# ysig/diff-mining

Measured on AMD Instinct MI355X. Metric: typicality-scored images/sec/node (512px, 10 t×2 prompts), higher is better.
Workload: dtype f16

## Files before the change

diff-mining_amd/csrc/igemm_pers_tr.hip:

```cpp
#include "igemm_pers_tile.h"

namespace dm {

namespace {

typedef volatile __attribute__((address_space(3))) int* lds_word_t;

template <int EXTRA, int WIMG, bool UNROLL = false, bool UP = false>
__global__ __launch_bounds__(512, 2)
void igemm_pers_tr_kernel(IGemmParams p, int ntiles, int cset) {
    constexpr int WC = 2, CH = 2, NW = 8;
    constexpr int TP = PERS_TP, TC = PERS_TC;
    constexpr int WBYTES = TC * 128;
    constexpr int PITCH = WIMG + 2;
    constexpr int IROWS = TP / WIMG;
    constexpr int ROWS = IROWS * PITCH;
    constexpr int XP = (ROWS + 7) / 8;
    constexpr int XBYTES = XP * 1024;
    constexpr int XI = (XP + NW - 1) / NW;
    constexpr int WI = TC / 8 / NW;
    constexpr int AUX_BYTES = 2048;
    constexpr bool GNBK = (EXTRA == PX_TEMB) && WIMG == 64;
    constexpr int NSTORE = pers_nstore(EPI_PLAIN, GNBK);
    static_assert(XI == 5 && 2 * WBYTES + 2 * XBYTES + 2 * AUX_BYTES <= 160 * 1024, "LDS budget");
    extern __shared__ __attribute__((aligned(16))) char smem[];
    char* const xs0 = smem + 2 * WBYTES;
    char* const aux0 = xs0 + 2 * XBYTES;

    const int wid = __builtin_amdgcn_readfirstlane(threadIdx.x >> 6);
    const int wc = wid % WC;
    const int wp = wid / WC;

    const int tiles_c = p.Cout / TC;
    int tile, tend, tdyn;
    const int xcd = blockIdx.x & 7;
    {
        const int nblk = gridDim.x;
        const int loc = blockIdx.x >> 3;
        const int tstart = xcd_range_start(blockIdx.x, ntiles);
        tend = tstart + (ntiles >> 3) + (xcd < (ntiles & 7) ? 1 : 0);
        tdyn = tstart + ((nblk - xcd + 7) >> 3);
        tile = tstart + loc;
    }
    int* const ctr = p.tile_ctr ? p.tile_ctr : &g_tile_ctr[cset][0];
    if (tile >= tend) { tiles_finish(ctr); return; }

    const int C1 = p.C1;
    const int C2 = p.Cin - C1;
    const int cpt = p.Cin / BK;
    const int ntrip = 3 * cpt;
    const int Ktot = 9 * p.Cin;
    const int OHW = p.OH * p.OW;

    int lp0 = 0, lc0 = 0;
    unsigned woff = 0;
    const unsigned wstride = (unsigned)(NW * 8) * (unsigned)Ktot;
    const f16* xbase = p.X;
    int ld_dy = 0, ld_cc = 0;

    auto set_wtile = [&](int tl) __attribute__((always_inline)) {
        const int pt = tl / tiles_c;
        lc0 = (tl - pt * tiles_c) * TC;
        const int ln = hw_lane();
        const int lrow = ln >> 3, lchunk = ((ln & 7) ^ lrow) * 8;
        woff = (unsigned)((size_t)(lc0 + wid * 8 + lrow) * Ktot + lchunk);
    };
    auto set_xtile = [&](int tl) __attribute__((always_inline)) {
        lp0 = (tl / tiles_c) * TP;
        ld_dy = 0; ld_cc = 0;
    };
    int x_dy = 0, x_cs = 0, x_cho = 0;
    auto src_pixel = [&](int i, int lrow) __attribute__((always_inline)) -> int {
        const int n = lp0 / OHW;
        const int oh0 = (lp0 - n * OHW) / WIMG;
        const int r = (wid + i * NW) * 8 + lrow;
        const int ir = r / PITCH;
        const int iw = r - ir * PITCH - 1;
        const int ih = oh0 + ir + x_dy - 1;
        if constexpr (UP) {
            const bool oku = r < ROWS && iw >= 0 && iw < WIMG && ih >= 0 && ih < p.OH;
            return oku ? (n * p.H + (ih >> 1)) * p.W + (iw >> 1) : -1;
        }
        const bool ok = r < ROWS && iw >= 0 && iw < WIMG && ih >= 0 && ih < p.H;
        return ok ? (n * p.H + ih) * WIMG + iw : -1;
    };
    auto prepare_x = [&]() __attribute__((always_inline)) {
        x_dy = ld_dy;
        const int ch = ld_cc * BK;
        if (ch < C1) { xbase = p.X; x_cs = C1; x_cho = ch; } else { xbase = p.X2; x_cs = C2; x_cho = ch - C1; }
        if (++ld_cc == cpt) { ld_cc = 0; ++ld_dy; }
    };
    auto load_w = [&](int buf, int idx, int adv) __attribute__((always_inline)) {
        lptr_t dst = (lptr_t)(smem + buf * WBYTES + (wid + idx * NW) * 1024);
        __builtin_amdgcn_global_load_lds((gptr_t)(p.Wp + (size_t)(woff + (unsigned)idx * wstride)), dst, 16, 0, 0);
        if (idx == WI - 1) woff += (unsigned)adv;
    };
    auto x_offset = [&](int i, int ln) __attribute__((always_inline)) -> int {
        const int lrow = ln >> 3, lchunk = ((ln & 7) ^ lrow) * 8;
        const int pix = src_pixel(i, lrow);
        return pix >= 0 ? pix * x_cs + x_cho + lchunk : -1;
    };
    auto load_x = [&](int buf, int i, int off, int ln) __attribute__((always_inline)) {
        if (i == XI - 1 && wid >= XP - NW * (XI - 1)) return;
        lptr_t dst = (lptr_t)(xs0 + buf * XBYTES + (wid + i * NW) * 1024);
        const f16* a = (off >= 0) ? (xbase + (size_t)(unsigned)off)
                                  : reinterpret_cast<const f16*>(p.zero_page) + lds_chunk(ln);
        __builtin_amdgcn_global_load_lds((gptr_t)a, dst, 16, 0, 0);
    };
    auto load_aux = [&](int slot, int lc0, int lp0) __attribute__((always_inline)) {
        char* ax = aux0 + slot * AUX_BYTES;
        const int lane = hw_lane();
        const char* zp = reinterpret_cast<const char*>(p.zero_page) + lane * 16;
        (void)load_aux_bias_temb<EXTRA>(p, ax, wid, lane, zp, lc0, lp0, OHW);
    };

    floatx4 acc[CH][5][4];

    constexpr bool SNAKE = DM_MFMA_SNAKE && !(EXTRA == PX_TEMB && WIMG == 64 && UNROLL);
    auto step = [&](int wcur, int xcur, auto dxv, int adv) __attribute__((always_inline)) {
        const int dx = dxv;
        const char* wt = smem + wcur * WBYTES;
        const char* xt = xs0 + xcur * XBYTES;
        const int ln = hw_lane();
        const int l15 = ln & 15, lg = ln >> 4;
        const int a_row_off = (wc * 80 * CH + l15) * 128;
        const int koff0 = ((lg ^ (l15 & 7)) << 4), koff1 = (((4 + lg) ^ (l15 & 7)) << 4);
        const int rb = ((wp * 64) / WIMG) * PITCH + (wp * 64) % WIMG + dx + l15;
        int boff[4];
#pragma unroll
        for (int j = 0; j < 4; ++j) {
            const int cj = ((16 * j) / WIMG) * PITCH + (16 * j) % WIMG;
            if (j > 0 && (cj & 7) == 0) { boff[j] = boff[0] + cj * 128; continue; }
            const int row = rb + cj;
            boff[j] = row * 128 + ((lg ^ (row & 7)) << 4);
        }
        half8 b0[4], b1[4], a[5];
#pragma unroll
        for (int j = 0; j < 4; ++j) b0[j] = *reinterpret_cast<const half8*>(xt + boff[j]);
#pragma unroll
        for (int i = 0; i < 5; ++i) a[i] = *reinterpret_cast<const half8*>(wt + a_row_off + i * 2048 + koff0);
        int grp = 0;
#pragma unroll
        for (int q = 0; q < 2 * CH; ++q) {
            const int sidx = q / CH, h = q % CH;
            if (q == CH - 1) {
#pragma unroll
                for (int j = 0; j < 4; ++j) {
                    const int cj = ((16 * j) / WIMG) * PITCH + (16 * j) % WIMG;
                    const int o1 = (j > 0 && (cj & 7) == 0) ? (boff[0] ^ 64) + cj * 128 : (boff[j] ^ 64);
                    b1[j] = *reinterpret_cast<const half8*>(xt + o1);
                }
            }
#pragma unroll
            for (int i = 0; i < 5; ++i) {
#pragma unroll
                for (int jj = 0; jj < 4; ++jj) {
                    const int j = (SNAKE && !(i & 1)) ? 3 - jj : jj;
                    acc[h][i][j] = __builtin_amdgcn_mfma_f32_16x16x32_f16(a[i], sidx ? b1[j] : b0[j], acc[h][i][j], 0, 0, 0);
                }
                if (q + 1 < 2 * CH) {
                    const int nq = q + 1, ns = nq / CH, nh = nq % CH;
                    a[i] = *reinterpret_cast<const half8*>(wt + a_row_off + nh * (80 * 128) + i * 2048 + (ns ? koff1 : koff0));
                }
                if (grp == 0) { load_w(wcur ^ 1, 0, adv); load_w(wcur ^ 1, 1, adv); }
                if (grp == 1) { load_w(wcur ^ 1, 2, adv); load_w(wcur ^ 1, 3, adv); }
                if (grp == 2) { load_w(wcur ^ 1, 4, adv); load_x(xcur ^ 1, 2 * dx, x_offset(2 * dx, ln), ln); }
                if (grp == 3) { if (dx < 2) load_x(xcur ^ 1, 2 * dx + 1, x_offset(2 * dx + 1, ln), ln); }
                ++grp;
                __builtin_amdgcn_sched_barrier(0);
            }
        }
    };

    set_wtile(tile);
    set_xtile(tile);
    load_aux(0, lc0, lp0);
    prepare_x();
    {
        const int ln = hw_lane();
#pragma unroll
        for (int i = 0; i < WI; ++i) load_w(0, i, p.Cin);
#pragma unroll
        for (int i = 0; i < XI; ++i) load_x(0, i, x_offset(i, ln), ln);
    }
    prepare_x();

    int g = 0;
    int tg = 0;
    int slot = 0;
    bool first = true;
    while (true) {
        const int pt = tile / tiles_c;
        const int p0 = pt * TP, c0out = (tile - pt * tiles_c) * TC;
#pragma unroll
        for (int h = 0; h < CH; ++h)
#pragma unroll
            for (int i = 0; i < 5; ++i)
#pragma unroll
                for (int j = 0; j < 4; ++j) acc[h][i][j] = floatx4{0.f, 0.f, 0.f, 0.f};

        if (first) wait_vmcnt_barrier<0>();
        else wait_vmcnt_barrier<NSTORE>();
        first = false;
        int ticket = 0;
        auto thread0 = [&]() __attribute__((always_inline)) -> bool {
            if constexpr (GNBK) return wid == 0 && hw_lane() == 0;
            else return threadIdx.x == 0;
        };
        if (thread0()) ticket = atomicAdd(&ctr[xcd * 32], 1);
        int next = 0;
        bool has_next = false;
        if constexpr (UNROLL) {
            int cc = 0;
            for (int tr = 0; tr < ntrip; ++tr) {
                const bool last = tr == ntrip - 1;
                step(g & 1, tg & 1, std::integral_constant<int, 0>{}, p.Cin);
                ++g;
                wait_vmcnt_barrier<0>();
                if (tr == 0 && thread0()) *ticket_word<lds_word_t, AUX_BYTES>(aux0, slot) = ticket;
                step(g & 1, tg & 1, std::integral_constant<int, 1>{}, (cc == cpt - 1) ? BK : BK - 2 * p.Cin);
                ++g;
                if (last) {
                    next = tdyn + *ticket_word<lds_word_t, AUX_BYTES>(aux0, slot);
                    next = __builtin_amdgcn_readfirstlane(next);
                    has_next = next < tend;
                    set_wtile(has_next ? next : tile);
                }
                wait_vmcnt_barrier<0>();
                step(g & 1, tg & 1, std::integral_constant<int, 2>{}, p.Cin);
                ++g;
                ++tg;
                if (tr == ntrip - 2) {
                    int nx = tdyn + *ticket_word<lds_word_t, AUX_BYTES>(aux0, slot);
                    nx = __builtin_amdgcn_readfirstlane(nx);
                    const bool hn = nx < tend;
                    set_xtile(hn ? nx : tile);
                    if (hn) load_aux(slot ^ 1, (nx - (nx / tiles_c) * tiles_c) * TC, lp0);
                }
                prepare_x();
                if (++cc == cpt) cc = 0;
                if (!last) wait_vmcnt_barrier<0>();
            }
        } else {
        const int nk = 3 * ntrip;
            int dx = 0, tr = 0, cc = 0;
            for (int kt = 0; kt < nk; ++kt) {
                const int adv = (dx == 1) ? ((cc == cpt - 1) ? BK : BK - 2 * p.Cin) : p.Cin;
                step(g & 1, tg & 1, dx, adv);
                ++g;
                if (dx == 1 && tr == ntrip - 1) {
                    next = tdyn + *ticket_word<lds_word_t, AUX_BYTES>(aux0, slot);
                    next = __builtin_amdgcn_readfirstlane(next);
                    has_next = next < tend;
                    set_wtile(has_next ? next : tile);
                }
                if (dx == 2) {
                    ++tg;
                    if (tr == ntrip - 2) {
                        int nx = tdyn + *ticket_word<lds_word_t, AUX_BYTES>(aux0, slot);
                        nx = __builtin_amdgcn_readfirstlane(nx);
                        const bool hn = nx < tend;
                        set_xtile(hn ? nx : tile);
                        if (hn) load_aux(slot ^ 1, (nx - (nx / tiles_c) * tiles_c) * TC, lp0);
                    }
                    prepare_x();
                    dx = 0; ++tr;
                    if (++cc == cpt) cc = 0;
                } else ++dx;
                if (kt < nk - 1) wait_vmcnt_barrier<0>();
                if (kt == 0 && thread0()) *ticket_word<lds_word_t, AUX_BYTES>(aux0, slot) = ticket;
            }
        }
        pers_epilogue<EPI_PLAIN, false, EXTRA, false, false, GNBK, AUX_BYTES>(p, acc, aux0, wid, wc, wp, p0, c0out, slot, 0);
        if (!has_next) break;
        tile = next;
        slot ^= 1;
    }
    tiles_finish(ctr);
}

}

#ifdef DM_TR_ALL_UNROLL
template <int EXTRA, int WIMG> struct TrUnroll { static constexpr bool value = true; };
#else
template <int EXTRA, int WIMG> struct TrUnroll { static constexpr bool value = false; };
#endif
#if !defined(DM_TR_NO_UNROLL) && !defined(DM_TR_ALL_UNROLL)
template <> struct TrUnroll<PX_NONE, 64> { static constexpr bool value = true; };
template <> struct TrUnroll<PX_TEMB, 64> { static constexpr bool value = true; };
template <> struct TrUnroll<PX_NONE, 128> { static constexpr bool value = true; };
template <> struct TrUnroll<PX_TEMB, 128> { static constexpr bool value = true; };
template <> struct TrUnroll<PX_TEMB, 32> { static constexpr bool value = true; };
template <> struct TrUnroll<PX_TEMB, 16> { static constexpr bool value = true; };
#endif

#ifndef DM_TR_UP_UNROLL
#define DM_TR_UP_UNROLL false
#endif
template <int EXTRA, int WIMG>
constexpr pers_kernel_t tr_kernel = igemm_pers_tr_kernel<EXTRA, WIMG, TrUnroll<EXTRA, WIMG>::value>;

template <int WIMG>
constexpr size_t tr_lds = 2 * (size_t)PERS_TC * 128 + 2 * (size_t)(((PERS_TP / WIMG) * (WIMG + 2) + 7) / 8) * 1024 + 2 * 2048;

template <int WIMG>
static hipError_t launch_tr_w(const IGemmParams& p, hipStream_t s) {
    static std::atomic<uint64_t> attr_seen{0};
    set_lds_once(attr_seen, tr_lds<WIMG>, {tr_kernel<PX_NONE, WIMG>, tr_kernel<PX_TEMB, WIMG>, tr_kernel<PX_RES, WIMG>});
    return launch_pers(p.temb ? tr_kernel<PX_TEMB, WIMG> : p.res ? tr_kernel<PX_RES, WIMG> : tr_kernel<PX_NONE, WIMG>,
                       tr_lds<WIMG>, (p.M / PERS_TP) * (p.Cout / PERS_TC), p, s);
}

static hipError_t launch_tr_up64(const IGemmParams& p, hipStream_t s) {
    static std::atomic<uint64_t> attr_seen{0};
    set_lds_once(attr_seen, tr_lds<64>, {igemm_pers_tr_kernel<PX_NONE, 64, DM_TR_UP_UNROLL, true>});
    return launch_pers(igemm_pers_tr_kernel<PX_NONE, 64, DM_TR_UP_UNROLL, true>, tr_lds<64>, (p.M / PERS_TP) * (p.Cout / PERS_TC), p, s);
}

bool igemm_pers_tr_ok(const IGemmParams& p) {
    if (p.Cout % 320 != 0 || p.M % 256 != 0 || p.Cin < 320 || (p.temb && p.res)) return false;
    const long long cmax = p.C1 > p.Cin - p.C1 ? p.C1 : p.Cin - p.C1;
    return (long long)p.M * cmax < (1ll << 31) && 9ll * p.Cin * p.Cout < (1ll << 31);
}

hipError_t launch_igemm_pers_tr(const IGemmParams& p, hipStream_t s) {
    if (!igemm_ko_layer(p) || !igemm_pers_tr_ok(p)) return hipErrorInvalidValue;
    if (p.mode == IG_CONV3_UP) return p.OW == 64 ? launch_tr_up64(p, s) : hipErrorInvalidValue;
    return p.OW == 128 ? launch_tr_w<128>(p, s) : p.OW == 64 ? launch_tr_w<64>(p, s) : p.OW == 32 ? launch_tr_w<32>(p, s) : launch_tr_w<16>(p, s);
}

}
```

Measured before the change: 61.67.

## Add lean address-generation path for residual 64-wide implicit GEMM conv kernel

After: 61.62. Within noise of the previous version (-0.1%).

```diff
diff --git a/diff-mining_amd/csrc/igemm_pers_tr.hip b/diff-mining_amd/csrc/igemm_pers_tr.hip
--- a/diff-mining_amd/csrc/igemm_pers_tr.hip
+++ b/diff-mining_amd/csrc/igemm_pers_tr.hip
@@ -1,10 +1,19 @@
 #include "igemm_pers_tile.h"
 
+#ifndef DM_TR_LEAN
+#define DM_TR_LEAN 1
+#endif
+
 namespace dm {
 
 namespace {
 
+typedef const __attribute__((address_space(3))) half8* lds_half8_t;
 typedef volatile __attribute__((address_space(3))) int* lds_word_t;
+
+constexpr bool tr_lean(int EXTRA, int WIMG, bool UP) {
+    return !UP && (DM_TR_LEAN == 2 || (DM_TR_LEAN == 1 && EXTRA == PX_RES && WIMG == 64));
+}
 
 template <int EXTRA, int WIMG, bool UNROLL = false, bool UP = false>
 __global__ __launch_bounds__(512, 2)
@@ -52,9 +61,15 @@
     const int Ktot = 9 * p.Cin;
     const int OHW = p.OH * p.OW;
 
+    constexpr bool LEAN = tr_lean(EXTRA, WIMG, UP);
+    constexpr bool WSCAL = LEAN && (!UNROLL || WIMG == 64);
     int lp0 = 0, lc0 = 0;
     unsigned woff = 0;
-    const unsigned wstride = (unsigned)(NW * 8) * (unsigned)Ktot;
+    const unsigned wstride = (unsigned)(NW * 8) * (unsigned)Ktot * (LEAN ? (unsigned)sizeof(f16) : 1u);
+    const char* wbase = reinterpret_cast<const char*>(p.Wp);
+    const char* xsb = nullptr;
+    unsigned xo = 0;
+    int x_edge = 0;
     const f16* xbase = p.X;
     int ld_dy = 0, ld_cc = 0;
 
@@ -63,7 +78,11 @@
         lc0 = (tl - pt * tiles_c) * TC;
         const int ln = hw_lane();
         const int lrow = ln >> 3, lchunk = ((ln & 7) ^ lrow) * 8;
-        woff = (unsigned)((size_t)(lc0 + wid * 8 + lrow) * Ktot + lchunk);
+        if constexpr (WSCAL) {
+            wbase = reinterpret_cast<const char*>(p.Wp + (size_t)(lc0 + wid * 8) * Ktot);
+            woff = (unsigned)(lrow * Ktot + lchunk) * (unsigned)sizeof(f16);
+        } else
+        woff = (unsigned)((size_t)(lc0 + wid * 8 + lrow) * Ktot + lchunk) * (LEAN ? (unsigned)sizeof(f16) : 1u);
     };
     auto set_xtile = [&](int tl) __attribute__((always_inline)) {
         lp0 = (tl / tiles_c) * TP;
@@ -85,27 +104,88 @@
         return ok ? (n * p.H + ih) * WIMG + iw : -1;
     };
     auto prepare_x = [&]() __attribute__((always_inline)) {
-        x_dy = ld_dy;
+        if constexpr (!LEAN) x_dy = ld_dy;
         const int ch = ld_cc * BK;
-        if (ch < C1) { xbase = p.X; x_cs = C1; x_cho = ch; } else { xbase = p.X2; x_cs = C2; x_cho = ch - C1; }
+        if constexpr (LEAN) {
+            if (ld_cc == 0 || ch == C1) {
+                const f16* src = p.X;
+                int cho = ch;
+                x_cs = C1;
+                if (ch >= C1) { src = p.X2; x_cs = C2; cho = ch - C1; }
+                const int n = lp0 / OHW;
+                const int oh0 = (lp0 - n * OHW) / WIMG;
+                x_edge = ((oh0 == 0 && ld_dy == 0) ? 1 : 0) | ((oh0 + IROWS == p.H && ld_dy == 2) ? 2 : 0);
+                const int ln = hw_lane();
+                const int lrow = ln >> 3, lchunk = ((ln & 7) ^ lrow) * 8;
+                const long long pix0 = (long long)(n * p.H + oh0 + ld_dy - 1) * WIMG + (wid * 8 - 1);
+                xsb = reinterpret_cast<const char*>(src) + (pix0 * x_cs + cho) * (long long)sizeof(f16);
+                xo = (unsigned)(lrow * x_cs + lchunk) * (unsigned)sizeof(f16);
+            } else xsb += BK * sizeof(f16);
+        } else {
+            if (ch < C1) { xbase = p.X; x_cs = C1; x_cho = ch; } else { xbase = p.X2; x_cs = C2; x_cho = ch - C1; }
+        }
         if (++ld_cc == cpt) { ld_cc = 0; ++ld_dy; }
     };
     auto load_w = [&](int buf, int idx, int adv) __attribute__((always_inline)) {
         lptr_t dst = (lptr_t)(smem + buf * WBYTES + (wid + idx * NW) * 1024);
-        __builtin_amdgcn_global_load_lds((gptr_t)(p.Wp + (size_t)(woff + (unsigned)idx * wstride)), dst, 16, 0, 0);
-        if (idx == WI - 1) woff += (unsigned)adv;
+        if constexpr (WSCAL) {
+            __builtin_amdgcn_global_load_lds((gptr_t)(wbase + (size_t)((unsigned)idx * wstride) + (size_t)woff), dst, 16, 0, 0);
+            if (idx == WI - 1) wbase += (long long)adv * (long long)sizeof(f16);
+        } else if constexpr (LEAN) {
+            __builtin_amdgcn_global_load_lds((gptr_t)(reinterpret_cast<const char*>(p.Wp) + (size_t)(woff + (unsigned)idx * wstride)), dst, 16, 0, 0);
+            if (idx == WI - 1) woff += (unsigned)adv * (unsigned)sizeof(f16);
+        } else {
+            __builtin_amdgcn_global_load_lds((gptr_t)(p.Wp + (size_t)(woff + (unsigned)idx * wstride)), dst, 16, 0, 0);
+            if (idx == WI - 1) woff += (unsigned)adv;
+        }
+    };
+    auto load_x_lean = [&](int buf, int i, int ln) __attribute__((always_inline)) {
+        if (i == XI - 1 && wid >= XP - NW * (XI - 1)) return;
+        lptr_t dst = (lptr_t)(xs0 + buf * XBYTES + (wid + i * NW) * 1024);
+        int w;
+        asm volatile("s_mov_b32 %0, %1" : "=s"(w) : "s"(wid));
+        const int rbase = (w + i * NW) * 8;
+        const int ira = rbase / PITCH;
+        const int t = (ira + 1) * PITCH - rbase;
+        const unsigned long long second = t < 8 ? ~0ull << (8 * t) : 0ull;
+        unsigned long long inv = t <= 8 ? 0xFFFFull << (8 * (t - 1)) : (t == PITCH ? 0xFFull : 0ull);
+        if constexpr (ROWS % 8 != 0) {
+            const int rem = ROWS - rbase;
+            if (rem < 8) inv |= ~0ull << (8 * rem);
+        }
+        if ((x_edge & 1) && ira == 0) inv |= ~second;
+        if (x_edge & 2) {
+            if (ira == IROWS - 1) inv |= ~second;
+            else if (ira == IROWS - 2) inv |= second;
+        }
+        const char* sb = xsb + (long long)((64 * i - 2 * ira) * x_cs) * (long long)sizeof(f16);
+        unsigned off = xo;
+        if (second != 0ull) {
+            sb -= 4 * x_cs;
+            off += __builtin_amdgcn_inverse_ballot_w64(second) ? 0u : (unsigned)(4 * x_cs);
+        }
+        if (inv == 0ull) __builtin_amdgcn_global_load_lds((gptr_t)(sb + (size_t)off), dst, 16, 0, 0);
+        else {
+            const char* a = sb + (size_t)off;
+            a = __builtin_amdgcn_inverse_ballot_w64(inv) ? reinterpret_cast<const char*>(p.zero_page) + (unsigned)(ln * 16) : a;
+            __builtin_amdgcn_global_load_lds((gptr_t)a, dst, 16, 0, 0);
+        }
     };
     auto x_offset = [&](int i, int ln) __attribute__((always_inline)) -> int {
         const int lrow = ln >> 3, lchunk = ((ln & 7) ^ lrow) * 8;
         const int pix = src_pixel(i, lrow);
         return pix >= 0 ? pix * x_cs + x_cho + lchunk : -1;
     };
-    auto load_x = [&](int buf, int i, int off, int ln) __attribute__((always_inline)) {
+    auto load_x_row = [&](int buf, int i, int off, int ln) __attribute__((always_inline)) {
         if (i == XI - 1 && wid >= XP - NW * (XI - 1)) return;
         lptr_t dst = (lptr_t)(xs0 + buf * XBYTES + (wid + i * NW) * 1024);
         const f16* a = (off >= 0) ? (xbase + (size_t)(unsigned)off)
                                   : reinterpret_cast<const f16*>(p.zero_page) + lds_chunk(ln);
         __builtin_amdgcn_global_load_lds((gptr_t)a, dst, 16, 0, 0);
+    };
+    auto load_x = [&](int buf, int i, int ln) __attribute__((always_inline)) {
+        if constexpr (LEAN) load_x_lean(buf, i, ln);
+        else load_x_row(buf, i, x_offset(i, ln), ln);
     };
     auto load_aux = [&](int slot, int lc0, int lp0) __attribute__((always_inline)) {
         char* ax = aux0 + slot * AUX_BYTES;
@@ -130,15 +210,25 @@
 #pragma unroll
         for (int j = 0; j < 4; ++j) {
             const int cj = ((16 * j) / WIMG) * PITCH + (16 * j) % WIMG;
+            if constexpr (LEAN) {
+                int jf = j;
+#pragma unroll
+                for (int e = j - 1; e >= 0; --e)
+                    if (((((16 * e) / WIMG) * PITCH + (16 * e) % WIMG) & 7) == (cj & 7)) jf = e;
+                if (jf != j) { boff[j] = boff[jf] + (cj - (((16 * jf) / WIMG) * PITCH + (16 * jf) % WIMG)) * 128; continue; }
+                boff[j] = (rb * 128 + (int)(unsigned)(size_t)(lptr_t)xt) + ((lg ^ ((rb + (cj & 7)) & 7)) << 4) + cj * 128;
+                continue;
+            }
             if (j > 0 && (cj & 7) == 0) { boff[j] = boff[0] + cj * 128; continue; }
             const int row = rb + cj;
             boff[j] = row * 128 + ((lg ^ (row & 7)) << 4);
         }
         half8 b0[4], b1[4], a[5];
 #pragma unroll
-        for (int j = 0; j < 4; ++j) b0[j] = *reinterpret_cast<const half8*>(xt + boff[j]);
+        for (int j = 0; j < 4; ++j) b0[j] = LEAN ? *reinterpret_cast<lds_half8_t>((size_t)(unsigned)boff[j]) : *reinterpret_cast<const half8*>(xt + boff[j]);
 #pragma unroll
         for (int i = 0; i < 5; ++i) a[i] = *reinterpret_cast<const half8*>(wt + a_row_off + i * 2048 + koff0);
+        const int aoff0 = (int)(unsigned)(size_t)(lptr_t)wt + a_row_off + koff0, aoff1 = aoff0 ^ 64;
         int grp = 0;
 #pragma unroll
         for (int q = 0; q < 2 * CH; ++q) {
@@ -147,8 +237,16 @@
 #pragma unroll
                 for (int j = 0; j < 4; ++j) {
                     const int cj = ((16 * j) / WIMG) * PITCH + (16 * j) % WIMG;
-                    const int o1 = (j > 0 && (cj & 7) == 0) ? (boff[0] ^ 64) + cj * 128 : (boff[j] ^ 64);
-                    b1[j] = *reinterpret_cast<const half8*>(xt + o1);
+                    int o1 = (j > 0 && (cj & 7) == 0) ? (boff[0] ^ 64) + cj * 128 : (boff[j] ^ 64);
+                    if constexpr (LEAN) {
+                        int jf = j;
+#pragma unroll
+                        for (int e = j - 1; e >= 0; --e)
+                            if (((((16 * e) / WIMG) * PITCH + (16 * e) % WIMG) & 7) == (cj & 7)) jf = e;
+                        const int cf = ((16 * jf) / WIMG) * PITCH + (16 * jf) % WIMG;
+                        o1 = ((boff[jf] - cf * 128) ^ 64) + cj * 128;
+                    }
+                    b1[j] = LEAN ? *reinterpret_cast<lds_half8_t>((size_t)(unsigned)o1) : *reinterpret_cast<const half8*>(xt + o1);
                 }
             }
 #pragma unroll
@@ -160,12 +258,13 @@
                 }
                 if (q + 1 < 2 * CH) {
                     const int nq = q + 1, ns = nq / CH, nh = nq % CH;
-                    a[i] = *reinterpret_cast<const half8*>(wt + a_row_off + nh * (80 * 128) + i * 2048 + (ns ? koff1 : koff0));
+                    a[i] = LEAN ? *reinterpret_cast<lds_half8_t>((size_t)(unsigned)((ns ? aoff1 : aoff0) + nh * (80 * 128) + i * 2048))
+                                : *reinterpret_cast<const half8*>(wt + a_row_off + nh * (80 * 128) + i * 2048 + (ns ? koff1 : koff0));
                 }
                 if (grp == 0) { load_w(wcur ^ 1, 0, adv); load_w(wcur ^ 1, 1, adv); }
                 if (grp == 1) { load_w(wcur ^ 1, 2, adv); load_w(wcur ^ 1, 3, adv); }
-                if (grp == 2) { load_w(wcur ^ 1, 4, adv); load_x(xcur ^ 1, 2 * dx, x_offset(2 * dx, ln), ln); }
-                if (grp == 3) { if (dx < 2) load_x(xcur ^ 1, 2 * dx + 1, x_offset(2 * dx + 1, ln), ln); }
+                if (grp == 2) { load_w(wcur ^ 1, 4, adv); load_x(xcur ^ 1, 2 * dx, ln); }
+                if (grp == 3) { if (dx < 2) load_x(xcur ^ 1, 2 * dx + 1, ln); }
                 ++grp;
                 __builtin_amdgcn_sched_barrier(0);
             }
@@ -181,7 +280,7 @@
 #pragma unroll
         for (int i = 0; i < WI; ++i) load_w(0, i, p.Cin);
 #pragma unroll
-        for (int i = 0; i < XI; ++i) load_x(0, i, x_offset(i, ln), ln);
+        for (int i = 0; i < XI; ++i) load_x(0, i, ln);
     }
     prepare_x();
 
@@ -287,12 +386,14 @@
 template <int EXTRA, int WIMG> struct TrUnroll { static constexpr bool value = false; };
 #endif
 #if !defined(DM_TR_NO_UNROLL) && !defined(DM_TR_ALL_UNROLL)
+template <> struct TrUnroll<PX_TEMB, 64> { static constexpr bool value = true; };
+template <> struct TrUnroll<PX_TEMB, 32> { static constexpr bool value = true; };
+#if DM_TR_LEAN != 2
 template <> struct TrUnroll<PX_NONE, 64> { static constexpr bool value = true; };
-template <> struct TrUnroll<PX_TEMB, 64> { static constexpr bool value = true; };
 template <> struct TrUnroll<PX_NONE, 128> { static constexpr bool value = true; };
 template <> struct TrUnroll<PX_TEMB, 128> { static constexpr bool value = true; };
-template <> struct TrUnroll<PX_TEMB, 32> { static constexpr bool value = true; };
 template <> struct TrUnroll<PX_TEMB, 16> { static constexpr bool value = true; };
+#endif
 #endif
 
 #ifndef DM_TR_UP_UNROLL
```
